# henryxrl/Listening-to-Sound-of-Silence-for-Speech-Denoising

Measured on AMD Instinct MI355X. Metric: utterances/sec (2 s clips), training step: detector + denoiser forward/backward/Adam, higher is better.
Workload: dtype fp16

## Files before the change

### listening-to-sound-of-silence-for-speech-denoising_amd/csrc/conv.hip

```cpp
#include "sos_common.h"
#include <stdlib.h>
#include <string.h>
#include <unistd.h>
#include <algorithm>
#include <array>
#include <map>
#include <type_traits>
#include <vector>

typedef sos_half_t bf16x8 __attribute__((ext_vector_type(8)));
typedef float f32x16 __attribute__((ext_vector_type(16)));

#ifdef SOS_ABLATE
#define CDBG(bit) (p.dbg & (bit))
#else
#define CDBG(bit) 0
#endif

struct ConvParams {
    const bf16_t* in;
    const bf16_t* wgt;
    void* out;
    const float* scale;
    const float* shift;
    const float* slope;
    const int* wgather;
    int B, H, W, Wl, in_cs, cin_off, cin, ktot, cps, seg_stride;
    int tT, tk, tpad;
    int kh, kw, cout, cout_pad, cout_store;
    int stride, dh, dw, pad_t, pad_l, pad_mode;
    int Ho, Wo;
    int out_dtype, c_off, act, accum;
    float* stats;
    int stats_c;
    const float* in_scale;
    const float* in_shift;
    const int* wl_tab;
    const int* wo_tab;
    int wg_stride;
    long long sb, sh, sw, sc, third;
    int NC, TH, TW, PH, PW;
    int nchunks;
    int npix;
    int tiles_h, tiles_w, ngw;
    int nblk;
    int lmap;
    int dbg;
    void* out2;
    int fP, fH, fW, fsy, foy, fsx, fox, frow;
    long long fthird;
    unsigned mgTW, mgTH, mgPW, mgPH, mg_tiles_w, mg_ngw, mg_tiles_h, mg_dh, mg_kw;
};

__host__ __device__ __forceinline__ unsigned mg_of(int d) { return d <= 1 ? 0u : (unsigned)((1ull << 32) / (unsigned)d + 1ull); }
__host__ __device__ __forceinline__ int mg_div(int n, unsigned mg) {
    return mg ? (int)(((unsigned long long)(unsigned)n * mg) >> 32) : n;
}
__host__ __device__ __forceinline__ void tile_decode_mg(int m, const ConvParams& p, int& cls, int& i, int& j) {
    const int r = mg_div(m, p.mgTW);
    j = m - r * p.TW;
    cls = mg_div(r, p.mgTH);
    i = r - cls * p.TH;
}

__host__ __device__ __forceinline__ void tile_decode(int m, int TH, int TW, int& cls, int& i, int& j) {
    const int r = m / TW;
    j = m - r * TW;
    cls = r / TH;
    i = r - cls * TH;
}

__device__ __forceinline__ bf16x8 lds_frag(const char* p) {
    return __builtin_bit_cast(bf16x8, *(const uint4*)p);
}

typedef __attribute__((address_space(3))) void* lds_ptr_t;

__device__ __forceinline__ void build_pixel_table(const ConvParams& p, unsigned* tab, int tid, int hin0, int win0, int rw0,
                                                  const int Wl, const int* __restrict__ wgather) {
    const bool reflect = p.pad_mode == SOS_PAD_REFLECT;
    for (int pix = tid; pix < p.npix; pix += 256) {
        const int rr = mg_div(pix, p.mgPW), c = pix - rr * p.PW;
        int r = rr, cls = 0;
        if (p.NC > 1) { cls = mg_div(rr, p.mgPH); r = rr - cls * p.PH; }
        int h = hin0 + r * p.dh;
        int w = win0 + cls * p.stride + c * p.dw;
        bool ok = (rw0 + cls) < p.dw || cls == 0;
        if (reflect) { h = reflect_index(h, p.H); w = reflect_index(w, Wl); }
        ok = ok && h >= 0 && h < p.H && w >= 0 && w < Wl;
        unsigned off = 0xffffffffu;
        if (ok) {
            if (wgather) w = wgather[w];
            off = (unsigned)((h * p.W + w) * p.in_cs) * 2u;
        }
        tab[pix] = off;
    }
}

template <int RP> struct StageMap {
    static constexpr int PPI = (64 / RP) * RP >= 56 ? 64 / RP : 0;
    static constexpr int LDS_STEP = PPI ? PPI * RP * 16 : 1024;
    int lp, lq;
    bool on;
    __device__ __forceinline__ StageMap(int lane) {
        lp = PPI ? lane / RP : 0;
        lq = PPI ? lane - lp * RP : 0;
        on = PPI ? lane < PPI * RP : true;
    }
    static __device__ __forceinline__ int ninstr(int npix) { return PPI ? (npix + PPI - 1) / PPI : (npix * RP + 63) >> 6; }
    __device__ __forceinline__ void at(int i, int lane, int& pix, int& q) const {
        if constexpr (PPI != 0) { pix = i * PPI + lp; q = lq; }
        else { const int L = i * 64 + lane; pix = L / RP; q = L - pix * RP; }
    }
    __device__ __forceinline__ bool writes(int i, int lane, int npix) const {
        if constexpr (PPI != 0) return i * PPI + lp < npix;
        else return i * 64 + lane < npix * RP;
    }
};

template <int CPR, bool PAD = true>
__device__ __forceinline__ void stage_patch_dma(const ConvParams& p, char* patch, unsigned tab_addr, int lane, int wave,
                                                __amdgpu_buffer_rsrc_t rsrc, unsigned cbytes, const int first = 0) {
    constexpr int RP = CPR + (PAD ? 1 : 0);
    typedef StageMap<RP> SM;
    const SM sm(lane);
    const int ninstr = SM::ninstr(p.npix);
    if (!sm.on) return;
    for (int i0 = first + wave; i0 < ninstr; i0 += 16) {
        unsigned ent[4], ta[4];
        int qq[4];
#pragma unroll
        for (int u = 0; u < 4; ++u) {
            int pix;
            sm.at(i0 + 4 * u, lane, pix, qq[u]);
            ta[u] = tab_addr + (unsigned)min(pix, p.npix - 1) * 4u;
        }
        asm volatile("ds_read_b32 %0, %4\n\tds_read_b32 %1, %5\n\tds_read_b32 %2, %6\n\tds_read_b32 %3, %7\n\ts_waitcnt lgkmcnt(0)"
                     : "=&v"(ent[0]), "=&v"(ent[1]), "=&v"(ent[2]), "=&v"(ent[3])
                     : "v"(ta[0]), "v"(ta[1]), "v"(ta[2]), "v"(ta[3])
                     : "memory");
#pragma unroll
        for (int u = 0; u < 4; ++u) {
            const int i = i0 + 4 * u;
            const bool ok = qq[u] < CPR && ent[u] != 0xffffffffu;
            const unsigned voff = ok ? ent[u] + cbytes + (unsigned)qq[u] * 16u : 0xffffffffu;
            if (i < ninstr && sm.writes(i, lane, p.npix))
                __builtin_amdgcn_raw_ptr_buffer_load_lds(rsrc, (lds_ptr_t)(patch + i * SM::LDS_STEP), 16, voff, 0, 0, 0);
        }
    }
}

#define SOS_STAGE_INVALID 0xfffe0000u
template <int CPR, bool PAD, int MAXR>
__device__ __forceinline__ void stage_prepare(const ConvParams& p, unsigned tab_addr, int lane, int wave, unsigned (&vb)[MAXR][4],
                                              unsigned& vlast) {
    constexpr int RP = CPR + (PAD ? 1 : 0);
    typedef StageMap<RP> SM;
    const SM sm(lane);
    const int ninstr = SM::ninstr(p.npix);
    auto resolve = [&](const int i) -> unsigned {
        int pix, q;
        sm.at(i, lane, pix, q);
        unsigned ent;
        asm volatile("ds_read_b32 %0, %1\n\ts_waitcnt lgkmcnt(0)" : "=&v"(ent) : "v"(tab_addr + (unsigned)min(pix, p.npix - 1) * 4u) : "memory");
        return (q < CPR && ent != 0xffffffffu && sm.writes(i, lane, p.npix)) ? ent + (unsigned)q * 16u : SOS_STAGE_INVALID;
    };
#pragma unroll
    for (int r = 0; r < MAXR; ++r) {
        const int i0 = wave + 16 * r;
        unsigned ent[4], ta[4];
// ... 247 lines not shown
                }
                hv = make_uint4(rh[0], rh[1], rh[2], rh[3]);
                lv = make_uint4(rl[0], rl[1], rl[2], rl[3]);
            }
            *(uint4*)(op + o) = hv;
            if (x3) {
                *(uint4*)(op + o + ith) = hv;
                *(uint4*)(op + o + 2 * ith) = lv;
            }
        } else {
            const bf16_t* hs = (const bf16_t*)(ost_hi + m * OROW + q * 16);
            const bf16_t* ls = (const bf16_t*)(ost_lo + m * OROW + q * 16);
            for (int e = 0; co + e < p.cout_store; ++e) {
                op[o + e] = hs[e];
                if (x3) { op[o + e + ith] = hs[e]; op[o + e + 2 * ith] = ls[e]; }
            }
        }
    }
}

#endif

template <int NT, int KS, bool SB, bool INBN = false, int PT = 2, bool W3 = false>
__global__ __launch_bounds__(256, (SB || W3) ? 3 : (PT > 2 ? 2 : 1)) void conv_mfma_kernel(ConvParams p) {
#if __HIP_DEVICE_COMPILE__
    constexpr int KC = 16 * KS;
    constexpr int PSTRIDE = KC * 2 + 16;
    constexpr int BSTRIDE = KC * 2 + 16;
    constexpr int CPR = 2 * KS;
    constexpr int BROWS = NT * 32;
    constexpr int BPIECES = BROWS * CPR;
    constexpr int NBREG = (BPIECES + 255) / 256;
    constexpr int BBYTES = SB ? BROWS * BSTRIDE : (BROWS * (CPR + 1) + 63) / 64 * 1024;
    extern __shared__ __attribute__((aligned(16))) char smem[];
    char* patch = smem;
    const int boff0 = p.npix * PSTRIDE;
    unsigned* pixtab = (unsigned*)(smem + boff0 + (SB ? 1 : 2) * BBYTES);

    const int tid = threadIdx.x;
    const int lane = tid & 63, wave = tid >> 6;
    const int l31 = lane & 31, lhi = lane >> 5;

    int bid = blockIdx.x;
    {
        const int nx = 8, q = p.nblk / nx, r = p.nblk % nx;
        const int xcd = bid % nx, loc = bid / nx;
        bid = (xcd < r ? xcd * (q + 1) : r * (q + 1) + (xcd - r) * q) + loc;
    }
    int t = bid, tq;
    tq = mg_div(t, p.mg_tiles_w); const int tj = t - tq * p.tiles_w; t = tq;
    tq = mg_div(t, p.mg_ngw); const int gw = t - tq * p.ngw; t = tq;
    tq = mg_div(t, p.mg_tiles_h); const int ti = t - tq * p.tiles_h; t = tq;
    tq = mg_div(t, p.mg_dh); const int rh = t - tq * p.dh; t = tq;
    const int b = t;
    const int n0 = blockIdx.y * BROWS;

    const int TH = p.TH, TW = p.TW;
    const int rw0 = gw * p.NC;
    const int ho_base = rh + ti * TH * p.dh;
    const int wo_base = rw0 + tj * TW * p.dw;
    const int hin0 = ho_base * p.stride - p.pad_t;
    const int win0 = wo_base * p.stride - p.pad_l;
    int Wl = p.Wl, Wo = p.Wo;
    if (p.wl_tab) {
        Wl = p.wl_tab[b]; Wo = p.wo_tab[b];
        if (wo_base >= Wo) return;
    }
    const int* wgather = p.wgather ? p.wgather + (long long)b * p.wg_stride : nullptr;

    int lpix = l31;
    if (p.lmap) {
        const bool g0 = l31 < 4 || (l31 >= 12 && l31 < 16) || (l31 >= 20 && l31 < 28);
        const int rank = g0 ? (l31 < 4 ? l31 : (l31 < 16 ? l31 - 8 : l31 - 12)) : (l31 < 12 ? l31 - 4 : (l31 < 20 ? l31 - 8 : l31 - 16));
        if (p.lmap == 1) lpix = (g0 ? 0 : 16) + rank;
        else lpix = ((g0 ? 0 : 1) + 2 * (rank >> 3)) * 8 + (rank & 7);
    }
    int abase[PT];
#pragma unroll
    for (int mt = 0; mt < PT; ++mt) {
        const int m = wave * (32 * PT) + mt * 32 + lpix;
        int cls, i, j;
        tile_decode_mg(m, p, cls, i, j);
        if (cls >= p.NC) cls = i = j = 0;
        abase[mt] = ((cls * p.PH + i * p.stride) * p.PW + j * p.stride) * PSTRIDE + lhi * 16;
    }
    const int bfrag_off = l31 * BSTRIDE + lhi * 16;

    int bsrc[NBREG], bdst[NBREG];
    {
        const int rmax = p.cout_pad - 1 - n0;
#pragma unroll
        for (int u = 0; u < NBREG; ++u) {
            const int idx = min(tid + u * 256, BPIECES - 1);
            const int row = idx / CPR, q = idx - row * CPR;
            bsrc[u] = min(row, rmax) * p.ktot + q * 8;
            bdst[u] = row * BSTRIDE + q * 16;
        }
    }
    const long long tap_stride = (long long)p.cout_pad * p.ktot;
    constexpr int RPB = CPR + 1;
    constexpr int WQ = BROWS * RPB;
    constexpr int WINSTR = (WQ + 63) / 64;
    constexpr int WPW = (WINSTR + 3) / 4;
    const int wv = __builtin_amdgcn_readfirstlane(wave);
    unsigned wvoff[WPW];
    {
        const int rmax = p.cout_pad - 1 - n0;
#pragma unroll
        for (int u = 0; u < WPW; ++u) {
            const int q = (wv + 4 * u) * 64 + lane;
            const int row = q / RPB, c = q - row * RPB;
            wvoff[u] = (c < CPR && row < BROWS) ? (unsigned)(((n0 + min(row, rmax)) * p.ktot + c * 8) * 2) : 0xffffffffu;
        }
    }
    const __amdgpu_buffer_rsrc_t w_rsrc = __builtin_amdgcn_make_buffer_rsrc(
        (void*)p.wgt, 0, (unsigned)((long long)p.kh * p.kw * p.cout_pad * p.ktot * 2), 0x00020000);
    auto dma_slab = [&](const int buf, const unsigned soff) {
#pragma unroll
        for (int u = 0; u < WPW; ++u) {
            const int i = wv + 4 * u;
            if (i < WINSTR)
                __builtin_amdgcn_raw_ptr_buffer_load_lds(w_rsrc, (lds_ptr_t)(smem + boff0 + buf * BBYTES + i * 1024), 16, wvoff[u],
                                                         soff, 0, 0);
        }
    };

    f32x16 acc[PT][NT];
#pragma unroll
    for (int mt = 0; mt < PT; ++mt)
#pragma unroll
        for (int nt = 0; nt < NT; ++nt)
#pragma unroll
            for (int e = 0; e < 16; ++e) acc[mt][nt][e] = 0.f;

    const int ntaps = p.kh * p.kw;
    const int tl_ = min(lane, ntaps - 1), ta_ = mg_div(tl_, p.mg_kw);
    const int tapoff = (ta_ * p.PW + (tl_ - ta_ * p.kw)) * PSTRIDE;
    const int tfr = b % p.tT;
    const long long frame_elems = (long long)p.H * p.W * p.in_cs;
    const long long in_b = (long long)(b - tfr) * p.H * p.W;
    const __amdgpu_buffer_rsrc_t in_rsrc =
        __builtin_amdgcn_make_buffer_rsrc((void*)(p.in + in_b * p.in_cs), 0, (unsigned)(p.tT * frame_elems) * 2u, 0x00020000);
    build_pixel_table(p, pixtab, tid, hin0, win0, rw0, Wl, wgather);
    constexpr int STG_R = 4;
    unsigned stg[STG_R][4], stg_last;
    const bool stg_fast = p.tk == 1;
    __syncthreads();
    if (stg_fast && !CDBG(1)) stage_prepare<CPR, true, STG_R>(p, (unsigned)(uintptr_t)pixtab, lane, __builtin_amdgcn_readfirstlane(wave), stg, stg_last);

    int seg = 0, cin_seg = 0;
    for (int cc = 0; cc < p.nchunks; ++cc) {
        if (cc) __syncthreads();
        if (!CDBG(1)) {
            if (stg_fast) {
                const unsigned cb = (unsigned)((p.cin_off + seg * p.seg_stride + cin_seg * KC) * 2);
                if constexpr (INBN) stage_issue_bn<CPR, STG_R>(p, patch, lane, __builtin_amdgcn_readfirstlane(wave), in_rsrc, cb, stg, stg_last, cin_seg * KC);
                else stage_issue<CPR, true, STG_R>(p, patch, (unsigned)(uintptr_t)pixtab, lane, __builtin_amdgcn_readfirstlane(wave), in_rsrc, cb, stg, stg_last);
            } else {
                const long long cbase = (long long)p.cin_off + (long long)(seg / p.tk) * p.seg_stride + (long long)cin_seg * KC +
                                        (long long)(tfr + seg % p.tk - p.tpad) * frame_elems;
                stage_patch_dma<CPR>(p, patch, (unsigned)(uintptr_t)pixtab, lane, __builtin_amdgcn_readfirstlane(wave), in_rsrc,
                                     (unsigned)(cbase * 2));
            }
        }
        if (++cin_seg == p.cps) { cin_seg = 0; ++seg; }
        if constexpr (!SB) dma_slab(0, (unsigned)(cc * KC * 2));
        else {
            const bf16_t* wsrc = p.wgt + ((long long)n0 * p.ktot + (long long)cc * KC);
#pragma unroll
            for (int u = 0; u < NBREG; ++u) {
                const uint4 v = *(const uint4*)(wsrc + bsrc[u]);
                if ((u + 1) * 256 <= BPIECES || tid + u * 256 < BPIECES) *(uint4*)(smem + boff0 + bdst[u]) = v;
            }
        }
        asm volatile("s_waitcnt vmcnt(0)" ::: "memory");
        __syncthreads();

        bf16x8 af[2][PT], wfr[2][NT];
#pragma unroll
        for (int mt = 0; mt < PT; ++mt) af[0][mt] = lds_frag(patch + abase[mt]);
        const bf16_t* wtap = p.wgt + ((long long)n0 * p.ktot + (long long)cc * KC);
        auto tap_body = [&](auto ftag, const int tap) {
            constexpr int F = decltype(ftag)::value;
            const int cur = SB ? 0 : (tap & 1);
            uint4 br0, br1, br2, br3, br4, br5, br6, br7;
            constexpr bool WD = !SB;
            if constexpr (WD) { if (tap + 1 < ntaps && !CDBG(8)) dma_slab(cur ^ 1, (unsigned)(((long long)(tap + 1) * tap_stride + cc * KC) * 2)); }
            if (tap + 1 < ntaps && !CDBG(64)) wtap += tap_stride;
#define SOS_BLOAD(i) if constexpr (NBREG > i && !WD) { if (!CDBG(8)) br##i = *(const uint4*)(wtap + bsrc[i]); else br##i = make_uint4(0,0,0,0); }
            SOS_BLOAD(0) SOS_BLOAD(1) SOS_BLOAD(2) SOS_BLOAD(3) SOS_BLOAD(4) SOS_BLOAD(5) SOS_BLOAD(6) SOS_BLOAD(7)
#undef SOS_BLOAD
            __builtin_amdgcn_sched_barrier(0);

            const int toff = __builtin_amdgcn_readlane(tapoff, tap);
            const int toffn = __builtin_amdgcn_readlane(tapoff, min(tap + 1, ntaps - 1));
            const char* ap[PT];
#pragma unroll
            for (int mt = 0; mt < PT; ++mt) ap[mt] = patch + abase[mt] + toff;
            const char* bp = smem + boff0 + cur * BBYTES + bfrag_off;
#pragma unroll
            for (int nt = 0; nt < NT; ++nt) wfr[F][nt] = lds_frag(bp + nt * 32 * BSTRIDE);
#pragma unroll
            for (int kk = 0; kk < KS; ++kk) {
                constexpr int dummy = 0; (void)dummy;
                const int cb = (F + kk) & 1, nb = cb ^ 1;
                if (kk + 1 < KS) {
#pragma unroll
                    for (int mt = 0; mt < PT; ++mt) af[nb][mt] = lds_frag(ap[mt] + (kk + 1) * 32);
#pragma unroll
                    for (int nt = 0; nt < NT; ++nt) wfr[nb][nt] = lds_frag(bp + nt * 32 * BSTRIDE + (kk + 1) * 32);
                } else {
#pragma unroll
                    for (int mt = 0; mt < PT; ++mt) af[nb][mt] = lds_frag(patch + abase[mt] + toffn);
                }
                __builtin_amdgcn_sched_barrier(0);
#pragma unroll
                for (int nt = 0; nt < NT; ++nt) {
#pragma unroll
                    for (int mt = 0; mt < PT; ++mt) acc[mt][nt] = SOS_MFMA_32x32x16(wfr[cb][nt], af[cb][mt], acc[mt][nt], 0, 0, 0);
                }
// ... 418 lines not shown
            const int po = (tap1[0] ? t1n : t0n) + coff[0];
#pragma unroll
            for (int pt = 0; pt < PT; ++pt) fbn[pt] = lds_frag(patch + pbase[pt] + po);
        }
#endif
#endif
        if constexpr (SB) {
            __syncthreads();
            if (w + 1 < nwin && !CDBG(8)) dma_window(w + 1, 0);
        }
        asm volatile("s_waitcnt vmcnt(0)" ::: "memory");
        __syncthreads();
    }
    }

    if (CDBG(4)) return;
    conv16_epilogue<NT16, PT>(p, acc, smem, tid, wave, l15, g, b, ho_base, wo_base, rw0, Wo);
#endif
}


static const size_t LDS_LIMIT = 160 * 1024;

typedef void (*conv_kernel_t)(ConvParams);

static inline int nseg_eff(const sos_conv_desc* d) { return d->in_nseg * (d->t_taps > 1 ? d->t_taps : 1); }

static int nt16_for(const sos_conv_desc* d) {
    const bool plain = d->in_nseg == 1 && d->out_dtype == SOS_DT_BF16, x3 = d->in_nseg == 3 && d->out_dtype == SOS_DT_BF16X3;
    if (!(plain || x3) || d->t_taps > 1 || d->out_sc != 1 || (d->cin != 16 && d->cin != 48)) return 0;
    if (d->cout <= 16) return 1;
    if (d->cout > 32 && d->cout <= 48) return 3;
    return 0;
}

static int nt_for(const sos_conv_desc* d) {
    const int ntiles = d->cout_pad / 32;
    const int nby = (ntiles + 3) / 4;
    return (ntiles + nby - 1) / nby;
}

struct ConvCfg {
    int NC, lth, ltw, ks;
    double cost;
};

static inline int tdim(int l) { return l < 16 ? 1 << l : l - 16; }
static inline int tenc(int v) {
    for (int l = 0; l < 16; ++l)
        if ((1 << l) == v) return l;
    return v + 16;
}

struct KsCode {
    bool row16;
    int nt;
    int ks;
    int nbuf;
    bool w3;
    int slots;
};
static KsCode decode(int ks, const sos_conv_desc* d) {
    if (ks <= 0) return {true, nt16_for(d), d->cin / 16, ks == 0 ? 2 : (ks == -1 ? 1 : 0), false, 256};
    KsCode v = {false, nt_for(d), 0, 2, false, 256};
    if (ks >= 1000) { v.nt = ks / 1000; ks %= 1000; }
    v.ks = ks % 100;
    switch (ks / 100) {
        case 0: break;
        case 1: v.nbuf = 1; break;
        case 2: v.w3 = true; break;
        case 3: v.slots = 384; break;
        default: v.nbuf = 0;
    }
    return v;
}

static size_t loop_lds(int npix, const KsCode& v) {
    const size_t row = (size_t)v.ks * 32 + (v.row16 ? 0 : 16);
    const size_t slab = v.row16 ? (v.nbuf == 1 ? (size_t)2 * v.nt * 16 * row : ((size_t)2 * v.nt * 16 * 2 * v.ks + 63) / 64 * 1024)
                                : (v.nbuf == 1 ? (size_t)v.nt * 32 * row : ((size_t)v.nt * 32 * (2 * v.ks + 1) + 63) / 64 * 1024);
    return (size_t)npix * row + v.nbuf * slab + (size_t)npix * 4;
}
static size_t loop_lds(const sos_conv_desc* d, int npix, int ks) { return loop_lds(npix, decode(ks, d)); }

struct ConvInstance {
    conv_kernel_t k;
    bool row16;
    int nt, ks, nbuf;
    bool w3;
    int slots;
    bool inbn;
};
#define SOS_K32(NT, KS, SB, INBN, PT, W3) {conv_mfma_kernel<NT, KS, SB, INBN, PT, W3>, false, NT, KS, (SB) ? 1 : 2, W3, 128 * (PT), INBN}
#define SOS_K32_DOUBLE(NT) SOS_K32(NT, 1, false, false, 2, false), SOS_K32(NT, 2, false, false, 2, false),                 \
    SOS_K32(NT, 3, false, false, 2, false), SOS_K32(NT, 4, false, false, 2, false), SOS_K32(NT, 5, false, false, 2, false), \
    SOS_K32(NT, 6, false, false, 2, false), SOS_K32(NT, 8, false, false, 2, false)
#define SOS_K32_SINGLE(NT) SOS_K32(NT, 1, true, false, 2, false), SOS_K32(NT, 2, true, false, 2, false),                   \
    SOS_K32(NT, 3, true, false, 2, false), SOS_K32(NT, 4, true, false, 2, false)
#define SOS_K16(NT16, KS) {conv16_kernel<NT16, KS, 0>, true, NT16, KS, 2, false, 256, false},                              \
    {conv16_kernel<NT16, KS, 1>, true, NT16, KS, 1, false, 256, false}
static const ConvInstance conv_instances[] = {
    SOS_K32_DOUBLE(1), SOS_K32_DOUBLE(2), SOS_K32_DOUBLE(3), SOS_K32_DOUBLE(4),
    SOS_K32_SINGLE(1), SOS_K32_SINGLE(2), SOS_K32_SINGLE(3),
    SOS_K32(3, 1, false, false, 2, true), SOS_K32(3, 2, false, false, 2, true),
    SOS_K32(3, 2, false, false, 3, false), SOS_K32(3, 3, false, false, 3, false),
    SOS_K32(3, 2, false, true, 2, false), SOS_K32(3, 3, false, true, 2, false),
    SOS_K16(1, 1), SOS_K16(1, 3), SOS_K16(3, 1), SOS_K16(3, 3),
};
#undef SOS_K16
#undef SOS_K32_SINGLE
#undef SOS_K32_DOUBLE
#undef SOS_K32

struct ConvPlan {
    conv_kernel_t k;
    dim3 grid;
    size_t lds;
    ConvParams p;
};
static const char* plan(const sos_conv_desc* d, const ConvCfg& c, ConvPlan* out);

static std::vector<ConvCfg> enumerate_cfgs(const sos_conv_desc* d, const char** why = nullptr) {
    std::vector<ConvCfg> out;
    const int nt = nt_for(d);
    const int Hc = (d->Ho + d->dil_h - 1) / d->dil_h, Wc = (d->Wo + d->dil_w - 1) / d->dil_w;
    const int taps = d->kh * d->kw;
    static const int kscand[] = {8, 6, 5, 4, 3, 2, 1};
    const int k16 = d->cin / 16;
    auto add_tile = [&](const int NC, const int TH, const int TW) {
        const int PH = (TH - 1) * d->stride + d->kh, PW = (TW - 1) * d->stride + d->kw;
        const int npix = NC * PH * PW;
        const long long th = (Hc + TH - 1) / TH, tw = (Wc + TW - 1) / TW, ngw = (d->dil_w + NC - 1) / NC;
        const double blocks = (double)th * tw * ngw * d->dil_h;
        if (nt16_for(d)) {
            for (int mode = 0; mode < 2; ++mode) {
                const size_t lds = loop_lds(d, npix, -mode);
                if (lds > LDS_LIMIT) continue;
                double per_block = 0.75 * nseg_eff(d) * (256.0 * taps * k16 + 3.0 * npix * k16 + 40.0 * (6 + taps / 2));
                if (lds > LDS_LIMIT / 2) per_block *= 1.3;
                else if (lds <= LDS_LIMIT / 3) per_block *= 0.95;
                out.push_back({NC, tenc(TH), tenc(TW), -mode, blocks * per_block});
            }
        }
        for (int ks : kscand) {
            if (k16 % ks) continue;
            const size_t lds = loop_lds(d, npix, ks);
            if (lds > LDS_LIMIT) continue;
            const int nchunks = nseg_eff(d) * k16 / ks;
            double per_block = 256.0 * taps * nchunks * ks + 3.0 * npix * nchunks * ks + 40.0 * nchunks * (6 + taps);
            if (lds > LDS_LIMIT / 2) per_block *= 1.3;
            out.push_back({NC, tenc(TH), tenc(TW), ks, blocks * per_block});
            const size_t lds1 = loop_lds(d, npix, ks + 100);
            if ((nt <= 2 ? ks <= 4 : (nt == 3 && ks <= 2)) && lds1 <= LDS_LIMIT / 3 && lds > LDS_LIMIT / 3)
                out.push_back({NC, tenc(TH), tenc(TW), ks + 100, blocks * per_block * 0.93});
            if (nt == 4) {
                const size_t lds2 = loop_lds(d, npix, ks + 2000);
                if (lds2 <= LDS_LIMIT / 2)
                    out.push_back({NC, tenc(TH), tenc(TW), ks + 2000, blocks * 2.0 * (128.0 * taps * nchunks * ks + 3.0 * npix * nchunks * ks + 40.0 * nchunks * (6 + taps)) * 0.9});
            }
        }
    };
    for (int lnc = 0; lnc <= 8; ++lnc) {
        const int NC = 1 << lnc;
        if (NC > 1 && (d->stride > 1 || NC > d->dil_w)) break;
        for (int lth = 0; lth + lnc <= 8; ++lth) add_tile(NC, 1 << lth, 1 << (8 - lnc - lth));
    }
    static const size_t LDS_THIRD = (LDS_LIMIT / 3) / 1280 * 1280;
    static const char* no_w3 = getenv("SOS_CONV_NO_W3");
    if (!(no_w3 && atoi(no_w3)) && nt == 3) {
        const size_t base = out.size();
        for (size_t i = 0; i < base; ++i) {
            const ConvCfg c = out[i];
            if (c.ks != 1 && c.ks != 2) continue;
            const int TH = tdim(c.lth), TW = tdim(c.ltw);
            const int PH = (TH - 1) * d->stride + d->kh, PW = (TW - 1) * d->stride + d->kw;
            if (loop_lds(d, c.NC * PH * PW, c.ks + 200) > LDS_THIRD || (size_t)256 * (3 * 64 + 16) > LDS_THIRD) continue;
            out.push_back({c.NC, c.lth, c.ltw, c.ks + 200, c.cost * 0.93});
        }
    }
    static const char* no_pt3 = getenv("SOS_CONV_NO_PT3");
    if (!(no_pt3 && atoi(no_pt3)) && nt == 3 && d->stride == 1) {
        static const int ncs[] = {1, 2, 3, 4, 6, 8, 12, 16, 24, 32}, ths[] = {1, 2, 3, 4, 6, 8, 12, 16, 24, 32, 48, 64};
        std::vector<std::array<int, 3>> seen;
        auto add384 = [&](const int NC, const int TH, const int TW) {
            if (NC < 1 || TH < 1 || TW < 2 || NC * TH * TW > 384 || NC * TH * TW < 300 || TH > 64 || TW > 64) return;
            const std::array<int, 3> t = {NC, TH, TW};
            if (std::find(seen.begin(), seen.end(), t) != seen.end()) return;
            seen.push_back(t);
            const int PH = TH - 1 + d->kh, PW = TW - 1 + d->kw;
            const int npix = NC * PH * PW;
            const long long th = (Hc + TH - 1) / TH, tw = (Wc + TW - 1) / TW, ngw = (d->dil_w + NC - 1) / NC;
            const double blocks = (double)th * tw * ngw * d->dil_h;
            for (int ks : {2, 3}) {
                if (k16 % ks) continue;
                const size_t stage = (size_t)384 * (3 * 64 + 16) + 384 * 4;
                const size_t lds = std::max(loop_lds(d, npix, ks + 300), stage);
                if (lds > LDS_LIMIT / 2) continue;
                const int nchunks = k16 / ks;
                const double per_block = 0.94 * 384.0 * taps * nchunks * ks + 3.0 * npix * nchunks * ks + 40.0 * nchunks * (6 + taps);
                out.push_back({NC, tenc(TH), tenc(TW), ks + 300, blocks * per_block});
            }
        };
        for (int NC : ncs) {
            if (NC > d->dil_w) break;
            const int ngw = (d->dil_w + NC - 1) / NC;
            if ((d->dil_w + ngw - 1) / ngw != NC) continue;
            for (int TH : ths) {
                if (TH > Hc && TH != ths[0]) { if (TH / 2 >= Hc) break; }
                const int THe = std::min(TH, Hc);
                const int TWmax = std::min(384 / (NC * THe), std::min(Wc, 64));
                add384(NC, THe, TWmax);
                if (TWmax >= 2) { const int parts = (Wc + TWmax - 1) / TWmax; add384(NC, THe, (Wc + parts - 1) / parts); }
                { const int parts = (Hc + THe - 1) / THe, THb = (Hc + parts - 1) / parts;
                  const int TWb = std::min(384 / (NC * THb), std::min(Wc, 64));
                  add384(NC, THb, TWb);
                  if (TWb >= 2) { const int pw = (Wc + TWb - 1) / TWb; add384(NC, THb, (Wc + pw - 1) / pw); } }
            }
        }
    }
    static const char* npot_env = getenv("SOS_CONV_NPOT");
    if (!(npot_env && atoi(npot_env) == 0) && d->stride == 1 && (Hc <= 48 || Wc <= 48)) {
        for (int ph = 1; ph <= 3; ++ph)
            for (int pw = 1; pw <= 3; ++pw) {
                const int TH = (Hc + ph - 1) / ph, TW = (Wc + pw - 1) / pw;
                if (TH < 1 || TW < 2 || TH * TW > 256 || TH > 64 || TW > 64) continue;
                int NC = 256 / (TH * TW);
                if (NC > d->dil_w) NC = d->dil_w;
                if (NC < 1) continue;
                const int ngw = (d->dil_w + NC - 1) / NC;
                NC = (d->dil_w + ngw - 1) / ngw;
                const bool pow2 = (TH & (TH - 1)) == 0 && (TW & (TW - 1)) == 0 && (NC & (NC - 1)) == 0 && NC * TH * TW == 256;
                if (pow2) continue;
                if (NC * TH * TW < 160) continue;
                add_tile(NC, TH, TW);
            }
    }
    const char* refused = nullptr;
    out.erase(std::remove_if(out.begin(), out.end(), [&](const ConvCfg& c) {
                  const char* r = plan(d, c, nullptr);
                  if (r && !refused) refused = r;
                  return r != nullptr;
              }), out.end());
    if (why) *why = refused;
    std::sort(out.begin(), out.end(), [](const ConvCfg& a, const ConvCfg& b) { return a.cost < b.cost; });
    return out;
}

struct ShapeKey {
    int v[19];
    bool operator<(const ShapeKey& o) const { return memcmp(v, o.v, sizeof(v)) < 0; }
};

static ShapeKey shape_key(const sos_conv_desc* d) {
    ShapeKey k;
    const int vals[19] = {d->B, d->H, d->W, d->Wl, d->cin, nseg_eff(d), d->cout_pad, d->kh, d->kw, d->stride, d->dil_h,
                          d->dil_w, d->Ho, d->Wo, d->out_dtype, d->out_sc == 1 ? 1 : 0, d->pad_mode, d->w_gather ? 1 : 0,
                          d->cout};
    memcpy(k.v, vals, sizeof(vals));
// ... 222 lines not shown

static int validate(const sos_conv_desc* d) {
    if (!d || !d->in || !d->wgt || !d->out || ((d->scale == nullptr) != (d->shift == nullptr))) {
        sos_set_error("sos_conv2d_fwd: null pointer");
        return SOS_EINVAL;
    }
    if (d->cin < 16 || d->cin % 16 || d->in_cs % 8 || d->cin_off % 8 || d->cout_pad % 32 || d->cout > d->cout_pad ||
        d->cout < 1 || d->kh < 1 || d->kw < 1 || d->kh * d->kw > 64 || d->stride < 1 || d->dil_h < 1 || d->dil_w < 1 ||
        (d->stride > 1 && (d->dil_h > 1 || d->dil_w > 1)) || d->B < 1 || d->Ho < 1 || d->Wo < 1 ||
        d->in_nseg < 1 || d->in_seg_stride % 8 || d->cin_off + (d->in_nseg - 1) * d->in_seg_stride + d->cin > d->in_cs ||
        d->cout_store < d->cout || d->out_dtype < 0 || d->out_dtype > 2 || (d->w_gather == nullptr && d->Wl != d->W)) {
        sos_set_error("sos_conv2d_fwd: bad descriptor (cin=%d in_cs=%d cin_off=%d cout=%d/%d k=%dx%d s=%d d=%dx%d)",
                      d->cin, d->in_cs, d->cin_off, d->cout, d->cout_pad, d->kh, d->kw, d->stride, d->dil_h, d->dil_w);
        return SOS_EINVAL;
    }
    if (d->t_taps > 1) {
        const long long frame_bytes = (long long)d->H * d->W * d->in_cs * 2;
        if (d->t_frames < 1 || d->B % d->t_frames || d->t_pad < 0 || d->t_pad >= d->t_taps || d->w_gather || d->wl_tab ||
            (d->t_frames + d->t_taps) * frame_bytes >= 0xffffff00ll) {
            sos_set_error("sos_conv2d_fwd: bad temporal taps (B=%d frames=%d taps=%d pad=%d; a clip plus the temporal halo "
                          "must stay below 4 GB)", d->B, d->t_frames, d->t_taps, d->t_pad);
            return SOS_EINVAL;
        }
    }
    if (d->stats && (d->out_dtype == SOS_DT_F32 || d->out_sc != 1 || d->stats_c < 1 || d->stats_c > d->cout_pad || d->accumulate)) {
        sos_set_error("sos_conv2d_fwd: fused statistics need a dense bf16 NHWC output without accumulation");
        return SOS_EINVAL;
    }
    if ((d->wl_tab == nullptr) != (d->wo_tab == nullptr) || (d->wl_tab && d->stats)) {
        sos_set_error("sos_conv2d_fwd: ragged batches need both wl_tab and wo_tab and no fused statistics");
        return SOS_EINVAL;
    }
    if ((d->in_scale == nullptr) != (d->in_shift == nullptr) ||
        (d->in_scale && (d->in_nseg != 1 || d->t_taps > 1 || d->cin % 8 || d->out_dtype == SOS_DT_BF16X3))) {
        sos_set_error("sos_conv2d_fwd: fused input BatchNorm needs in_scale AND in_shift, one 16-bit channel segment, no temporal taps");
        return SOS_EINVAL;
    }
    if ((long long)d->in_cs * 2 > 0xffff) {
        sos_set_error("sos_conv2d_fwd: pixel pitch of %d channels not supported (<= 32767)", d->in_cs);
        return SOS_EINVAL;
    }
    if ((uint64_t)d->H * d->W * d->in_cs * 2 >= 0xfff00000ull) {
        sos_set_error("sos_conv2d_fwd: one input image exceeds 4 GB");
        return SOS_ENOSPC;
    }
    if (d->fold_pad < 0 || (d->fold_pad > 0 && (!d->fold_pad_out || d->fold_H < 1 || d->fold_W < 1 || d->fold_sy < 1 || d->fold_sx < 1 ||
                                               d->fold_oy < 0 || d->fold_ox < 0 || d->fold_row < d->cout_store || d->fold_row % 8 ||
                                               d->out_dtype == SOS_DT_F32 || d->out_sc != 1 || d->stats || d->wl_tab ||
                                               (d->Ho - 1) * d->fold_sy + d->fold_oy >= d->fold_H + 2 * d->fold_pad ||
                                               (d->Wo - 1) * d->fold_sx + d->fold_ox >= d->fold_W + 2 * d->fold_pad ||
                                               (int64_t)(d->fold_H + 2 * d->fold_pad) * (d->fold_W + 2 * d->fold_pad) * d->fold_row >= 0x7ffffff0ll ||
                                               (int64_t)d->fold_H * d->fold_W * d->out_sw >= 0x7ffffff0ll))) {
        sos_set_error("sos_conv2d_fwd: bad reflection-pad fold (16-bit dense NHWC outputs inside the padded domain only)");
        return SOS_EINVAL;
    }
    if (d->out_dtype != SOS_DT_F32 && d->out_sc == 1 && !d->fold_pad &&
        (int64_t)(d->Ho - 1) * d->out_sh + (int64_t)(d->Wo - 1) * d->out_sw + d->out_c_off + d->cout_store >= 0x7ffffff0ll) {
        sos_set_error("sos_conv2d_fwd: one output image spans more than 2^31 elements (Ho=%d Wo=%d)", d->Ho, d->Wo);
        return SOS_ENOSPC;
    }
    if (d->pad_mode == SOS_PAD_REFLECT && (d->pad_top >= d->H || d->pad_left >= d->Wl)) {
        sos_set_error("sos_conv2d_fwd: reflect pad %d/%d needs a larger input (%dx%d)", d->pad_top, d->pad_left, d->H, d->Wl);
        return SOS_EINVAL;
    }
    return SOS_OK;
}

static int pick_lane_map(const ConvParams& p, int pstride) {
    static const int grp[2][16] = {{0, 1, 2, 3, 12, 13, 14, 15, 20, 21, 22, 23, 24, 25, 26, 27},
                                   {4, 5, 6, 7, 8, 9, 10, 11, 16, 17, 18, 19, 28, 29, 30, 31}};
    const int TW = p.TW, TH = p.TH;
    int best = 0, best_cost = 1 << 30;
    for (int mode = 0; mode < 3; ++mode) {
        if (mode == 2 && TW != 8) continue;
        int cost = 0;
        for (int g = 0; g < 2; ++g) {
            int cnt[16] = {0}, worst = 0;
            for (int k = 0; k < 16; ++k) {
                const int l = grp[g][k];
                const int lp = mode == 0 ? l : (mode == 1 ? g * 16 + k : (g + 2 * (k >> 3)) * 8 + (k & 7));
                int cls, i, j;
                tile_decode(lp, TH, TW, cls, i, j);
                if (cls >= p.NC) cls = i = j = 0;
                const int off = ((cls * p.PH + i * p.stride) * p.PW + j * p.stride) * pstride;
                worst = std::max(worst, ++cnt[(off >> 4) & 15]);
            }
            cost += worst;
        }
        if (cost < best_cost) { best_cost = cost; best = mode; }
    }
    return best;
}

static const char* plan(const sos_conv_desc* d, const ConvCfg& c, ConvPlan* out) {
    KsCode v = decode(c.ks, d);
    const int TH = tdim(c.lth), TW = tdim(c.ltw);
    if (c.NC < 1 || TH < 1 || TW < 1 || c.NC * TH * TW > v.slots) return "the pixel tile does not fit the workgroup";
    if (v.row16 ? !v.nt : (v.ks < 1 || d->cin % (16 * v.ks))) return "no kernel takes this shape with these k-steps";
    const bool x3 = d->out_dtype == SOS_DT_BF16X3, staged = d->out_dtype != SOS_DT_F32 && d->out_sc == 1;
    const bool dense16 = d->out_dtype == SOS_DT_BF16 && d->out_sc == 1 && nseg_eff(d) == 1 && d->cout_store % 8 == 0;
    if (v.w3 && (!dense16 || d->accumulate)) return "three workgroups per CU need a dense 16-bit output of whole 8-channel pieces, no accumulation";
    if (v.slots == 384 && (!dense16 || d->wl_tab)) return "384-slot tiles need a dense 16-bit output of whole 8-channel pieces, no ragged batch";
    const int PH = (TH - 1) * d->stride + d->kh, PW = (TW - 1) * d->stride + d->kw, npix = c.NC * PH * PW;
    if (v.row16) {
        static const char* e = getenv("SOS_CONV16_MODE");
        KsCode m = v;
        if (e && (atoi(e) == 0 || atoi(e) == 1)) m.nbuf = atoi(e) == 1 ? 1 : 2;
        if (loop_lds(npix, m) <= LDS_LIMIT) v = m;
    }
    const ConvInstance* inst = nullptr;
    for (const ConvInstance& i : conv_instances)
        if (i.row16 == v.row16 && i.nt == v.nt && i.ks == v.ks && i.nbuf == v.nbuf && i.w3 == v.w3 && i.slots == v.slots &&
            i.inbn == (d->in_scale != nullptr))
            inst = &i;
    if (!inst) return d->in_scale ? "fused input BatchNorm (in_scale) is built for three n-tiles, 2 or 3 k-steps, two slab buffers only"
                                  : "no kernel instance is built for this tiling";
    size_t lds = loop_lds(npix, v);
    if (v.row16 || staged) {
        const size_t orow = v.row16 ? (size_t)v.nt * 32 + 16 : (size_t)v.nt * 64 + 16, slots = v.slots;
        const size_t stage = v.w3 ? slots * orow
                                  : slots * orow * (x3 ? 2 : 1) + slots * 4 + ((d->stats && slots == 256) ? 16384 : 0);
        lds = std::max(lds, stage);
    }
    if (lds > LDS_LIMIT) return "the tile needs more LDS than a CU has";
    const int Hc = (d->Ho + d->dil_h - 1) / d->dil_h, Wc = (d->Wo + d->dil_w - 1) / d->dil_w;
    const int tiles_h = (Hc + TH - 1) / TH, tiles_w = (Wc + TW - 1) / TW, ngw = (d->dil_w + c.NC - 1) / c.NC;
    const long long nblk = (long long)d->B * d->dil_h * tiles_h * ngw * tiles_w;
    if (nblk > 0x7fffffffLL || nblk * std::max(std::max(tiles_w, ngw), std::max(tiles_h, (int)d->dil_h)) >= (1ll << 32))
        return "grid too large";
    if (!out) return nullptr;

    ConvParams& p = out->p;
    p.in = (const bf16_t*)d->in; p.wgt = (const bf16_t*)d->wgt; p.out = d->out;
    p.scale = d->scale; p.shift = d->shift; p.slope = d->act_param; p.wgather = d->w_gather;
    p.B = d->B; p.H = d->H; p.W = d->W; p.Wl = d->Wl; p.in_cs = d->in_cs; p.cin_off = d->cin_off; p.cin = d->cin;
    p.kh = d->kh; p.kw = d->kw; p.cout = d->cout; p.cout_pad = d->cout_pad; p.cout_store = d->cout_store;
    p.stride = d->stride; p.dh = d->dil_h; p.dw = d->dil_w; p.pad_t = d->pad_top; p.pad_l = d->pad_left;
    p.pad_mode = d->pad_mode; p.Ho = d->Ho; p.Wo = d->Wo; p.out_dtype = d->out_dtype; p.c_off = d->out_c_off;
    p.stats = d->stats; p.stats_c = d->stats_c;
    p.in_scale = d->in_scale; p.in_shift = d->in_shift;
    p.wl_tab = d->wl_tab; p.wo_tab = d->wo_tab; p.wg_stride = d->w_gather_stride;
    p.act = d->act; p.accum = d->accumulate; p.sb = d->out_sb; p.sh = d->out_sh; p.sw = d->out_sw; p.sc = d->out_sc; p.third = d->out_third;
    p.out2 = d->fold_pad_out; p.fP = d->fold_pad; p.fH = d->fold_H; p.fW = d->fold_W; p.fsy = d->fold_sy; p.foy = d->fold_oy;
    p.fsx = d->fold_sx; p.fox = d->fold_ox; p.frow = d->fold_row; p.fthird = d->fold_third;
    p.NC = c.NC; p.TH = TH; p.TW = TW; p.PH = PH; p.PW = PW; p.npix = npix;
    p.cps = v.row16 ? 1 : d->cin / (16 * v.ks);
    p.nchunks = p.cps * nseg_eff(d);
    p.ktot = d->cin * nseg_eff(d);
    p.tk = d->t_taps > 1 ? d->t_taps : 1; p.tT = d->t_taps > 1 ? d->t_frames : 1; p.tpad = d->t_taps > 1 ? d->t_pad : 0;
    p.seg_stride = d->in_seg_stride;
    p.tiles_h = tiles_h; p.tiles_w = tiles_w; p.ngw = ngw; p.nblk = (int)nblk;
    p.mgTW = mg_of(TW); p.mgTH = mg_of(TH); p.mgPW = mg_of(PW); p.mgPH = mg_of(PH);
    p.mg_tiles_w = mg_of(tiles_w); p.mg_ngw = mg_of(ngw); p.mg_tiles_h = mg_of(tiles_h); p.mg_dh = mg_of(d->dil_h); p.mg_kw = mg_of(d->kw);
    { const char* e = getenv("SOS_CONV_DBG"); p.dbg = e ? atoi(e) : 0; }
    p.lmap = 0;
    if (!v.row16) {
        static const char* nomap = getenv("SOS_CONV_NO_LANE_MAP");
        if (!nomap) p.lmap = pick_lane_map(p, v.ks * 32 + 16);
    }
    out->k = inst->k;
    out->grid = dim3((unsigned)nblk, v.row16 ? 1u : (unsigned)((d->cout_pad / 32 + v.nt - 1) / v.nt));
    out->lds = lds;
#ifdef SOS_ABLATE
    { static const char* e = getenv("SOS_CONV_LDS_PAD"); if (e) out->lds = std::min(out->lds + (size_t)atoi(e), LDS_LIMIT); }
#endif
    return nullptr;
}

static int launch_plan(const ConvPlan& pl, hipStream_t s) {
    static sos_device_once attr_once;
    const int arc = sos_per_device_once(attr_once, [] {
        for (const ConvInstance& i : conv_instances) {
            const hipError_t e = hipFuncSetAttribute((const void*)i.k, hipFuncAttributeMaxDynamicSharedMemorySize, (int)LDS_LIMIT);
            if (e != hipSuccess) {
                sos_set_error("sos_conv2d_fwd: hipFuncSetAttribute failed: %s", hipGetErrorString(e));
                return (int)SOS_ELAUNCH;
            }
        }
        return (int)SOS_OK;
    });
    if (arc) return arc;
    hipLaunchKernelGGL(pl.k, pl.grid, dim3(256), pl.lds, s, pl.p);
    return sos_check_launch("sos_conv2d_fwd");
}

static int launch_cfg(const sos_conv_desc* d, const ConvCfg& c, hipStream_t s) {
    ConvPlan pl;
    if (const char* why = plan(d, c, &pl)) {
        sos_set_error("sos_conv2d_fwd: tiling NC=%d TH=%d TW=%d ks=%d: %s", c.NC, tdim(c.lth), tdim(c.ltw), c.ks, why);
        return SOS_EINVAL;
    }
    return launch_plan(pl, s);
}

static long long tiles_of(const sos_conv_desc* d, const ConvCfg& c) {
    const int Hc = (d->Ho + d->dil_h - 1) / d->dil_h, Wc = (d->Wo + d->dil_w - 1) / d->dil_w;
    const int TH = tdim(c.lth), TW = tdim(c.ltw);
    return (long long)d->B * d->dil_h * ((Hc + TH - 1) / TH) * ((d->dil_w + c.NC - 1) / c.NC) * ((Wc + TW - 1) / TW);
}

static int resolve(const sos_conv_desc* d, const char* who, ConvCfg* c, ConvPlan* pl) {
    auto take = [&](const ConvCfg& e) {
        if (plan(d, e, pl)) return false;
        *c = e;
        return true;
    };
    auto take_entry = [&](const ConvCfg& e) { return take(e) || (decode(e.ks, d).w3 && take({e.NC, e.lth, e.ltw, e.ks - 200, 0.0})); };
    static const char* fpt3 = getenv("SOS_CONV_FORCE_PT3");
    static const char* fw3 = getenv("SOS_CONV_FORCE_W3");
    const bool pt3 = fpt3 && atoi(fpt3), w3 = fw3 && atoi(fw3);
    ConvCfg e;
    if ((pt3 || w3) && first_offered(d, [&](const ConvCfg& x) { const KsCode v = decode(x.ks, d); return (pt3 && v.slots == 384) || (w3 && v.w3); }, &e) &&
        take(e))
        return SOS_OK;
    static const char* force = getenv("SOS_CONV_FORCE_CFG");
    if (!force) {
        const ShapeKey k = shape_key(d);
        if (tuned_lookup(k, &e) && take_entry(e)) return SOS_OK;
        if (tuned_borrow(k, &e) && take_entry(e)) return SOS_OK;
    }
    const char* why = nullptr;
    const std::vector<ConvCfg> cfgs = enumerate_cfgs(d, &why);
    if (cfgs.empty()) {
        if (why) sos_set_error("%s: no tiling runs this descriptor: %s", who, why);
        else sos_set_error("%s: no tile fits LDS (cin=%d k=%dx%d)", who, d->cin, d->kh, d->kw);
        return why ? SOS_EINVAL : SOS_ENOSPC;
    }
    const size_t pick = force ? (size_t)atol(force) % cfgs.size() : 0;
    if (getenv("SOS_CONV_LIST"))
        fprintf(stderr, "%s: cfg %zu/%zu NC=%d TH=%d TW=%d ks=%d\n", who, pick, cfgs.size(), cfgs[pick].NC, tdim(cfgs[pick].lth),
                tdim(cfgs[pick].ltw), cfgs[pick].ks);
    take(cfgs[pick]);
    return SOS_OK;
}

extern "C" int64_t sos_conv2d_tile_count(const sos_conv_desc* d) {
// ... 142 lines not shown
```

Measured before the change: 561.4.

## Store strided-conv input patch in phase-split column order in LDS

For strided convolutions on the non-row16 path, the LDS input patch columns are reordered by stride phase, so columns with the same residue modulo the stride sit next to each other. The pixel table, A-fragment base offsets, tap offsets and the bank-conflict lane-map cost model all use the new column mapping. Adjacent output pixels then read contiguous LDS rows instead of rows spaced by the stride, which is meant to cut LDS bank conflicts. The patch pitch is rounded up to a multiple of the stride, which uses slightly more LDS and can change the tile choice. An environment variable disables the new layout.

Result: no change. 560.2 (median of 2 runs) (-0.2%).

```diff
diff --git a/listening-to-sound-of-silence-for-speech-denoising_amd/csrc/conv.hip b/listening-to-sound-of-silence-for-speech-denoising_amd/csrc/conv.hip
--- a/listening-to-sound-of-silence-for-speech-denoising_amd/csrc/conv.hip
+++ b/listening-to-sound-of-silence-for-speech-denoising_amd/csrc/conv.hip
@@ -50,7 +50,13 @@
     int fP, fH, fW, fsy, foy, fsx, fox, frow;
     long long fthird;
     unsigned mgTW, mgTH, mgPW, mgPH, mg_tiles_w, mg_ngw, mg_tiles_h, mg_dh, mg_kw;
+    int PWh;
+    unsigned mgPWh;
 };
+
+__host__ __device__ __forceinline__ int patch_col(const ConvParams& p, const int c) {
+    return p.PWh ? (c % p.stride) * p.PWh + c / p.stride : c;
+}
 
 __host__ __device__ __forceinline__ unsigned mg_of(int d) { return d <= 1 ? 0u : (unsigned)((1ull << 32) / (unsigned)d + 1ull); }
 __host__ __device__ __forceinline__ int mg_div(int n, unsigned mg) {
@@ -80,12 +86,18 @@
                                                   const int Wl, const int* __restrict__ wgather) {
     const bool reflect = p.pad_mode == SOS_PAD_REFLECT;
     for (int pix = tid; pix < p.npix; pix += 256) {
-        const int rr = mg_div(pix, p.mgPW), c = pix - rr * p.PW;
+        const int rr = mg_div(pix, p.mgPW);
+        int c = pix - rr * p.PW;
         int r = rr, cls = 0;
         if (p.NC > 1) { cls = mg_div(rr, p.mgPH); r = rr - cls * p.PH; }
+        bool ok = (rw0 + cls) < p.dw || cls == 0;
+        if (p.PWh) {
+            const int run = mg_div(c, p.mgPWh);
+            c = (c - run * p.PWh) * p.stride + run;
+            ok = ok && c < (p.TW - 1) * p.stride + p.kw;
+        }
         int h = hin0 + r * p.dh;
         int w = win0 + cls * p.stride + c * p.dw;
-        bool ok = (rw0 + cls) < p.dw || cls == 0;
         if (reflect) { h = reflect_index(h, p.H); w = reflect_index(w, Wl); }
         ok = ok && h >= 0 && h < p.H && w >= 0 && w < Wl;
         unsigned off = 0xffffffffu;
@@ -499,7 +511,7 @@
         int cls, i, j;
         tile_decode_mg(m, p, cls, i, j);
         if (cls >= p.NC) cls = i = j = 0;
-        abase[mt] = ((cls * p.PH + i * p.stride) * p.PW + j * p.stride) * PSTRIDE + lhi * 16;
+        abase[mt] = ((cls * p.PH + i * p.stride) * p.PW + patch_col(p, j * p.stride)) * PSTRIDE + lhi * 16;
     }
     const int bfrag_off = l31 * BSTRIDE + lhi * 16;
 
@@ -552,7 +564,7 @@
 
     const int ntaps = p.kh * p.kw;
     const int tl_ = min(lane, ntaps - 1), ta_ = mg_div(tl_, p.mg_kw);
-    const int tapoff = (ta_ * p.PW + (tl_ - ta_ * p.kw)) * PSTRIDE;
+    const int tapoff = (ta_ * p.PW + patch_col(p, tl_ - ta_ * p.kw)) * PSTRIDE;
     const int tfr = b % p.tT;
     const long long frame_elems = (long long)p.H * p.W * p.in_cs;
     const long long in_b = (long long)(b - tfr) * p.H * p.W;
@@ -1137,6 +1149,15 @@
     return (size_t)npix * row + v.nbuf * slab + (size_t)npix * 4;
 }
 static size_t loop_lds(const sos_conv_desc* d, int npix, int ks) { return loop_lds(npix, decode(ks, d)); }
+
+static bool phase_patch(const sos_conv_desc* d, const bool row16) {
+    static const char* e = getenv("SOS_CONV_NO_PHASE");
+    return !row16 && d->stride > 1 && !(e && atoi(e));
+}
+static int patch_pitch(const sos_conv_desc* d, const int TW, const bool phase) {
+    const int PW = (TW - 1) * d->stride + d->kw;
+    return phase ? (PW + d->stride - 1) / d->stride * d->stride : PW;
+}
 
 struct ConvInstance {
     conv_kernel_t k;
@@ -1185,6 +1206,7 @@
     auto add_tile = [&](const int NC, const int TH, const int TW) {
         const int PH = (TH - 1) * d->stride + d->kh, PW = (TW - 1) * d->stride + d->kw;
         const int npix = NC * PH * PW;
+        const int npix32 = NC * PH * patch_pitch(d, TW, phase_patch(d, false));
         const long long th = (Hc + TH - 1) / TH, tw = (Wc + TW - 1) / TW, ngw = (d->dil_w + NC - 1) / NC;
         const double blocks = (double)th * tw * ngw * d->dil_h;
         if (nt16_for(d)) {
@@ -1199,17 +1221,17 @@
         }
         for (int ks : kscand) {
             if (k16 % ks) continue;
-            const size_t lds = loop_lds(d, npix, ks);
+            const size_t lds = loop_lds(d, npix32, ks);
             if (lds > LDS_LIMIT) continue;
             const int nchunks = nseg_eff(d) * k16 / ks;
             double per_block = 256.0 * taps * nchunks * ks + 3.0 * npix * nchunks * ks + 40.0 * nchunks * (6 + taps);
             if (lds > LDS_LIMIT / 2) per_block *= 1.3;
             out.push_back({NC, tenc(TH), tenc(TW), ks, blocks * per_block});
-            const size_t lds1 = loop_lds(d, npix, ks + 100);
+            const size_t lds1 = loop_lds(d, npix32, ks + 100);
             if ((nt <= 2 ? ks <= 4 : (nt == 3 && ks <= 2)) && lds1 <= LDS_LIMIT / 3 && lds > LDS_LIMIT / 3)
                 out.push_back({NC, tenc(TH), tenc(TW), ks + 100, blocks * per_block * 0.93});
             if (nt == 4) {
-                const size_t lds2 = loop_lds(d, npix, ks + 2000);
+                const size_t lds2 = loop_lds(d, npix32, ks + 2000);
                 if (lds2 <= LDS_LIMIT / 2)
                     out.push_back({NC, tenc(TH), tenc(TW), ks + 2000, blocks * 2.0 * (128.0 * taps * nchunks * ks + 3.0 * npix * nchunks * ks + 40.0 * nchunks * (6 + taps)) * 0.9});
             }
@@ -1228,7 +1250,7 @@
             const ConvCfg c = out[i];
             if (c.ks != 1 && c.ks != 2) continue;
             const int TH = tdim(c.lth), TW = tdim(c.ltw);
-            const int PH = (TH - 1) * d->stride + d->kh, PW = (TW - 1) * d->stride + d->kw;
+            const int PH = (TH - 1) * d->stride + d->kh, PW = patch_pitch(d, TW, phase_patch(d, false));
             if (loop_lds(d, c.NC * PH * PW, c.ks + 200) > LDS_THIRD || (size_t)256 * (3 * 64 + 16) > LDS_THIRD) continue;
             out.push_back({c.NC, c.lth, c.ltw, c.ks + 200, c.cost * 0.93});
         }
@@ -1617,7 +1639,7 @@
                 int cls, i, j;
                 tile_decode(lp, TH, TW, cls, i, j);
                 if (cls >= p.NC) cls = i = j = 0;
-                const int off = ((cls * p.PH + i * p.stride) * p.PW + j * p.stride) * pstride;
+                const int off = ((cls * p.PH + i * p.stride) * p.PW + patch_col(p, j * p.stride)) * pstride;
                 worst = std::max(worst, ++cnt[(off >> 4) & 15]);
             }
             cost += worst;
@@ -1636,7 +1658,8 @@
     const bool dense16 = d->out_dtype == SOS_DT_BF16 && d->out_sc == 1 && nseg_eff(d) == 1 && d->cout_store % 8 == 0;
     if (v.w3 && (!dense16 || d->accumulate)) return "three workgroups per CU need a dense 16-bit output of whole 8-channel pieces, no accumulation";
     if (v.slots == 384 && (!dense16 || d->wl_tab)) return "384-slot tiles need a dense 16-bit output of whole 8-channel pieces, no ragged batch";
-    const int PH = (TH - 1) * d->stride + d->kh, PW = (TW - 1) * d->stride + d->kw, npix = c.NC * PH * PW;
+    const bool phase = phase_patch(d, v.row16);
+    const int PH = (TH - 1) * d->stride + d->kh, PW = patch_pitch(d, TW, phase), npix = c.NC * PH * PW;
     if (v.row16) {
         static const char* e = getenv("SOS_CONV16_MODE");
         KsCode m = v;
@@ -1687,6 +1710,7 @@
     p.tiles_h = tiles_h; p.tiles_w = tiles_w; p.ngw = ngw; p.nblk = (int)nblk;
     p.mgTW = mg_of(TW); p.mgTH = mg_of(TH); p.mgPW = mg_of(PW); p.mgPH = mg_of(PH);
     p.mg_tiles_w = mg_of(tiles_w); p.mg_ngw = mg_of(ngw); p.mg_tiles_h = mg_of(tiles_h); p.mg_dh = mg_of(d->dil_h); p.mg_kw = mg_of(d->kw);
+    p.PWh = phase ? PW / d->stride : 0; p.mgPWh = mg_of(p.PWh);
     { const char* e = getenv("SOS_CONV_DBG"); p.dbg = e ? atoi(e) : 0; }
     p.lmap = 0;
     if (!v.row16) {
```
